# panuelosj/polystokes

Measured on AMD Instinct MI355X. Metric: Stokes-solve wall ms/step (assembly+PCG) on 256^3 grid; CG iters/sec, lower is better.
Workload: dtype f64; 1 GPU; synthetic lid-driven cavity 256x256x256, reduced tiles (tile=16, pad=2), jacobi-PCG, tol 1e-3; parallelism=1 GPU

## Files before the change

### polystokes_amd/__init__.py

```python
import ctypes as C
import os
import subprocess

import numpy as np

from . import _abi
from ._abi import (FieldsIn, FieldsOut, Params, Scene, Stats, default_params)

_HERE = os.path.dirname(os.path.abspath(__file__))
LIB_PATH = os.environ.get("PS_LIB") or os.path.join(_HERE, "libpolystokes_hip.so")
_lib = None

EXPORTED_SYMBOLS = [
    "ps_abi_version", "ps_reduced_dof", "ps_context_create", "ps_context_destroy", "ps_last_error", "ps_params_default",
    "ps_upload_fields", "ps_step_device", "ps_setup_device", "ps_solve_device", "ps_download_fields",
    "polystokes_step", "ps_apply_operator", "ps_apply_preconditioner", "ps_query_array", "ps_read_array",
    "ps_export_component_matrices", "ps_export_matrices", "ps_export_stats", "ps_bench_kernel", "ps_memory_stats", "ps_set_interrupt", "ps_solve_exported_system",
    "ps_set_slab", "ps_set_brick", "ps_comm_unique_id", "ps_comm_init_rccl", "ps_comm_selftest", "ps_comm_init_tcp", "ps_dist_stats",
    "ps_group_create", "ps_group_destroy", "ps_group_rank", "ps_group_step",
    "ps_set_warm_start", "ps_download_solution_fields", "ps_upload_density_field", "ps_set_surface_tension",
    "ps_set_solid_boundary", "ps_set_rheology", "ps_set_solve_precision",
    "ps_upload_fields_device", "ps_upload_density_field_device", "ps_download_fields_device", "ps_download_solution_fields_device",
    "ps_step_device_fields",
]
# ... 144 lines not shown
        put = lambda a: _hip.DeviceBuffer.from_numpy(to_layout(a, layout), pad)
        self.layout, self.host = layout, scene
        for k in ("nx", "ny", "nz", "dx", "dt", "density", "name", "surface_tension"):
            setattr(self, k, getattr(scene, k))
        self.vel = [put(a) for a in scene.vel]
        self.collisionvel = [put(a) for a in scene.collisionvel]
        self.surface, self.collision, self.viscosity = put(scene.surface), put(scene.collision), put(scene.viscosity)
        self.weights = None if scene.weights is None else [put(a) for a in scene.weights]
        self.density_field = None if scene.density_field is None else put(scene.density_field)


def device_scene(scene, layout=_abi.LAYOUT_X_FASTEST, pad=0):
    return DeviceScene(scene, layout, pad)


def fields_in_device(fields):
    fi = FieldsIn()
    fi.nx, fi.ny, fi.nz = fields.nx, fields.ny, fields.nz
    fi.dx, fi.dt = fields.dx, fields.dt
    fi.orig[0] = fi.orig[1] = fi.orig[2] = 0.0
    fi.density = fields.density
    cv = getattr(fields, "collisionvel", None)
    for a in range(3):
        fi.vel[a] = device_address(fields.vel[a])
        fi.collisionvel[a] = device_address(cv[a]) if cv is not None else None
    fi.surface, fi.collision, fi.viscosity = (device_address(fields.surface), device_address(fields.collision),
                                              device_address(fields.viscosity))
    w = getattr(fields, "weights", None)
    for i in range(14):
        fi.weights[i] = device_address(w[i]) if w is not None else None
    return fi


_DT = {(1, "i"): np.int8, (4, "i"): np.int32, (4, "f"): np.float32, (8, "f"): np.float64, (4, "u"): np.uint32}


def _kind(name):
    if name.endswith(("Labels", "Indices", ".col", ".ptr", "Region", "Perm", ".chunkInfo", ".chunkRep", ".code")) or name.startswith("faceRow"):
        return "i"
    if name in ("valuesCoded", "columns16", "diagonalsCoded", "fusedStep", "streamRuns", "rowPerLane", "chebInner32", "warmStartUsed", "densityField", "launchWalk",
                "surfaceTensionReducedFaces", "solidBoundary", "solidSlipEdges", "rheologyModel", "rheologyIterations",
                "solvePrecisionUsed", "solvePassIterations"):
        return "i"
    if name in ("ownedX", "ownedY", "ownedZ"):
        return "f"
    if False:
        return "i"
    if name == "reducedRowFace":
        return "u"
    return "f"


def process_memory_stats():
    v = (C.c_int64 * 4)()
    lib().ps_memory_stats(None, v)
    return {"live_bytes": int(v[0]), "peak_bytes": int(v[1]), "contexts": int(v[3])}


class PolyStokesError(RuntimeError):
    pass


class Solver:

    def __init__(self, device=0, _handle=None):
        self.L = lib()
        self._owned = _handle is None
        h = self.L.ps_context_create(device) if _handle is None else _handle
        if not h:
            raise PolyStokesError(self.L.ps_last_error(None).decode())
        self.h = C.c_void_p(h)
        self.stats = Stats()
        self.scene = None

    def close(self):
        if getattr(self, "h", None):
            if self._owned:
                self.L.ps_context_destroy(self.h)
            self.h = None

    def set_interrupt(self, fn):
# ... 366 lines not shown
```

### polystokes_amd/csrc/ps_blocks.hip

```cpp
#include "ps_context.hpp"
#include "ps_setup_util.hpp"

using namespace ps;

namespace {

constexpr int BS = SETUP_BS;

struct BlockArgs {
    Grid g;
    double invDx;
    const float* lw[7];
    const float* fw[7];
    const int32_t* lab[7];
    const int32_t* act[7];
    const int32_t* reg[7];
    const int32_t* sys[7];
    const int32_t* sysT[3];
    const int32_t* faceRow[3];
    const float* vel[3];
    const float* cvel[3];
    CellField visc;
    FaceDensity dens;
    int64_t nP, nA, faceOff[3];
// ... 72 lines not shown

__device__ inline int skinFaceLen(const BlockArgs& A, int axis, int r, int i, int j, int k) {
    const int3 fd = A.g.dims(1 + axis);
    if (oob3(fd, i, j, k)) return 0;
    const int64_t c = lin3(fd, i, j, k);
    if (A.reg[1 + axis][c] != r || A.lab[1 + axis][c] != PS_REDUCED) return 0;
    int32_t cols[8];
    double vals[8];
    return faceEntries(A, axis, make_int3(i, j, k), cols, vals);
}
__device__ inline unsigned long long blockScanExclPacked(unsigned long long v, unsigned long long* total) {
    __shared__ unsigned long long waveSums64[BS / 64];
    const int lane = threadIdx.x & 63, w = threadIdx.x >> 6;
    unsigned long long incl = v;
#pragma unroll
    for (int o = 1; o < 64; o <<= 1) {
        const unsigned lo = __shfl_up((unsigned)(incl & 0xffffffffull), o, 64), hi = __shfl_up((unsigned)(incl >> 32), o, 64);
        if (lane >= o) incl += ((unsigned long long)hi << 32) | lo;
    }
    if (lane == 63) waveSums64[w] = incl;
    __syncthreads();
    unsigned long long base = 0, tot = 0;
#pragma unroll
    for (int i = 0; i < BS / 64; ++i) { if (i < w) base += waveSums64[i]; tot += waveSums64[i]; }
    __syncthreads();
    *total = tot;
    return base + incl - v;
}
constexpr int SKIN_LONG_MIN = 3;
template <bool ASSIGN>
__global__ void __launch_bounds__(BS) k_skin(BlockArgs A, const int32_t* __restrict__ bbox, const int32_t* __restrict__ itemRegion,
                                             const int32_t* __restrict__ itemStart, int32_t* __restrict__ itemCount, int32_t* __restrict__ faceRow0,
                                             int32_t* __restrict__ faceRow1, int32_t* __restrict__ faceRow2, uint32_t* __restrict__ rrowFace,
                                             int32_t* __restrict__ rrowRegion, int32_t* __restrict__ itemLong) {
    __shared__ unsigned char codes[ASSIGN ? FB_CHUNK : 1];
    const int item = blockIdx.x;
    const int r = itemRegion[item], start = itemStart[item];
    if (A.regionOwned && !A.regionOwned[r]) {
        if (!ASSIGN && threadIdx.x == 0) itemCount[item] = 0;
        if (ASSIGN && threadIdx.x == 0) itemLong[item] = 0;
        return;
    }
    const int bx0 = bbox[r * 6 + 0], by0 = bbox[r * 6 + 1], bz0 = bbox[r * 6 + 2];
    const int ex = bbox[r * 6 + 3] - bx0 + 2, ey = bbox[r * 6 + 4] - by0 + 2, ez = bbox[r * 6 + 5] - bz0 + 2;
    const int total = ex * ey * ez;
    const int end = min(start + FB_CHUNK, total);
    unsigned long long mine = 0;
    for (int base = start; base < end; base += BS) {
        const int pos = base + threadIdx.x;
        if (pos < end) {
            const int i = bx0 + pos % ex, j = by0 + (pos / ex) % ey, k = bz0 + pos / (ex * ey);
            int code = 0;
#pragma unroll
            for (int a = 0; a < 3; ++a) {
                const int n = skinFaceLen(A, a, r, i, j, k);
                if (n > 0) { const bool lg = n >= SKIN_LONG_MIN; code |= (lg ? 2 : 1) << (2 * a); mine += 1ull << (10 * ((lg ? 0 : 3) + a)); }
            }
            if (ASSIGN) codes[pos - start] = (unsigned char)code;
        }
    }
    int catBase[6] = {0, 0, 0, 0, 0, 0};
    if (ASSIGN) {
        int itemTot[6] = {0, 0, 0, 0, 0, 0};
        for (int base = start; base < end; base += BS) {
            const int pos = base + threadIdx.x;
            unsigned long long v = 0;
            if (pos < end) {
                const int code = codes[pos - start];
#pragma unroll
                for (int a = 0; a < 3; ++a) { const int q = (code >> (2 * a)) & 3; if (q) v += 1ull << (10 * ((q == 2 ? 0 : 3) + a)); }
            }
            unsigned long long bt;
            blockScanExclPacked(v, &bt);
#pragma unroll
            for (int c = 0; c < 6; ++c) itemTot[c] += (int)((bt >> (10 * c)) & 1023ull);
        }
        int run = itemCount[item];
#pragma unroll
        for (int c = 0; c < 6; ++c) { catBase[c] = run; run += itemTot[c]; }
        if (threadIdx.x == 0) itemLong[item] = itemTot[0] + itemTot[1] + itemTot[2];
        for (int base = start; base < end; base += BS) {
            const int pos = base + threadIdx.x;
            unsigned long long v = 0;
            int code = 0;
            if (pos < end) {
                code = codes[pos - start];
#pragma unroll
                for (int a = 0; a < 3; ++a) { const int q = (code >> (2 * a)) & 3; if (q) v += 1ull << (10 * ((q == 2 ? 0 : 3) + a)); }
            }
            unsigned long long bt;
            const unsigned long long off = blockScanExclPacked(v, &bt);
// ... 227 lines not shown
    const double visc = (double)A.visc.sample(A.g, (float)q.x + ox, (float)q.y + oy, (float)q.z + oz);
    const double invVisc = clampd(1. / visc, 0., 1e10);
    uInv[t] = A.own.sample(4 + ea, q.x, q.y, q.z) ? 2. * invVisc * vw : 0.;
    if (uDiag) uDiag[t] = 0.5 * visc * clampd(1. / vw, 0., 1.e2);
}

BlockArgs makeArgs(ps_context* c) {
    BlockArgs A;
    A.g = c->g; A.invDx = c->invDx;
    for (int s = 0; s < 7; ++s) {
        A.lw[s] = c->liquidW[s].p; A.fw[s] = c->fluidW[s].p;
        A.lab[s] = c->labels[s].p; A.act[s] = c->activeIdx[s].p; A.reg[s] = c->reducedIdx[s].p; A.sys[s] = c->sysIdx[s].p;
    }
    for (int a = 0; a < 3; ++a) { A.faceRow[a] = c->faceRow[a].p; A.vel[a] = c->vel[a].p; A.cvel[a] = c->cvel[a].p; A.sysT[a] = c->sysIdxT[a].p; }
    A.visc = c->viscSource(); A.dens = c->densSource();
    A.nP = c->nPressures; A.nA = c->nActiveVs;
    A.faceOff[0] = 0; A.faceOff[1] = c->nFace[0]; A.faceOff[2] = c->nFace[0] + c->nFace[1];
    A.own = c->own();
    A.valScale = c->valScale;
    A.codeFail = c->counters.p + CTR_CODE_FAIL;
    A.regionOwned = (c->slabEnabled && c->regionCount > 0) ? c->regionOwned.p : nullptr;
    A.freeSlip = c->solidBoundaryUsed == PS_SOLID_FREE_SLIP ? 1 : 0;
    A.slipEdges = A.freeSlip ? c->slipEdges.p : nullptr;
    return A;
}

__global__ void k_chunk_len4(const int32_t* __restrict__ ptr, const int2* __restrict__ chunkRows, int nChunks, int32_t* __restrict__ len4, int32_t* __restrict__ maxLen) {
    const int ch = blockIdx.x * blockDim.x + threadIdx.x;
    if (ch > nChunks) return;
    int n = 0;
    if (ch < nChunks) { const int2 cr = chunkRows[ch]; n = ptr[cr.x + cr.y] - ptr[cr.x]; atomicMax(maxLen, n); }
    len4[ch] = (n + 3) & ~3;
}
__global__ void __launch_bounds__(BS) k_col16_build(const int32_t* __restrict__ ptr, const int32_t* __restrict__ col, const int8_t* __restrict__ code,
                                                    const int2* __restrict__ chunkRows, const int32_t* __restrict__ start4, uint16_t* __restrict__ col16,
                                                    int8_t* __restrict__ code4, int32_t* __restrict__ winBase, int4* __restrict__ chunkInfo,
                                                    uint8_t* __restrict__ len8, int32_t* __restrict__ fail, int32_t* __restrict__ chunkRep, int nChunks) {
    const int lane = threadIdx.x & 63;
    const int chunk = blockIdx.x * (BS / 64) + (int)(threadIdx.x >> 6);
    if (chunk >= nChunks) return;
    if (lane == 0) chunkRep[chunk] = chunk;
    const int2 cr = chunkRows[chunk];
    const int r0 = cr.x;
    const int p0 = ptr[r0], p1 = ptr[r0 + cr.y];
    const int q0 = start4[chunk], q1 = start4[chunk + 1];
    if (lane == 0) chunkInfo[chunk] = make_int4(q0, (p1 - p0) | (cr.y << 16), cr.x, cr.x);
    for (int i = lane; i < cr.y; i += 64) len8[r0 + i] = (uint8_t)(ptr[r0 + i + 1] - ptr[r0 + i]);
    constexpr int SL = 32;
    if (p1 - p0 > SL * 64) { if (lane == 0) *fail = 1; return; }
    int c[SL];
    unsigned open = 0u;
#pragma unroll
    for (int u = 0; u < SL; ++u) {
        const int i = lane + u * 64;
        const bool o = p0 + i < p1;
        c[u] = o ? col[p0 + i] : 0x7fffffff;
        if (o) open |= 1u << u;
        if (q0 + i < q1) { code4[q0 + i] = o ? code[p0 + i] : (int8_t)0; if (!o) col16[q0 + i] = 0; }
    }
    int used = 16;
    for (int w = 0; w < 16; ++w) {
        int m = 0x7fffffff;
#pragma unroll
        for (int u = 0; u < SL; ++u) if ((open >> u) & 1u) m = min(m, c[u]);
        for (int o = 32; o > 0; o >>= 1) m = min(m, __shfl_xor(m, o));
        const int base = m;
        if (base == 0x7fffffff) { used = w; break; }
        if (lane == 0) winBase[(int64_t)chunk * 16 + w] = base;
#pragma unroll
        for (int u = 0; u < SL; ++u)
            if (((open >> u) & 1u) && c[u] - base < 4096) {
                col16[q0 + lane + u * 64] = (uint16_t)((w << 12) | (c[u] - base));
                open &= ~(1u << u);
            }
    }
    if (lane == 0) for (int w = used; w < 16; ++w) winBase[(int64_t)chunk * 16 + w] = 0;
    if (open) *fail = 1;
}
__global__ void __launch_bounds__(64) k_chunk_hash(const int4* __restrict__ chunkInfo, const uint16_t* __restrict__ col16, const int8_t* __restrict__ code4,
                                                   const uint8_t* __restrict__ len8, unsigned long long* __restrict__ hash, int weak) {
    const int chunk = blockIdx.x;
    const int4 ci = chunkInfo[chunk];
    const int n4 = ((ci.y & 0xffff) + 3) & ~3, rows = (int)((unsigned)ci.y >> 16);
    unsigned long long h = 0;
    if (!weak)
    for (int i = threadIdx.x; i < n4; i += 64)
        h += mix64(((unsigned long long)i << 32) | ((unsigned long long)col16[ci.x + i] << 8) | (uint8_t)code4[ci.x + i]);
    if (!weak)
    for (int i = threadIdx.x; i < rows; i += 64) h += mix64(0x4000000000000000ull | ((unsigned long long)i << 32) | len8[ci.z + i]);
    for (int o = 32; o > 0; o >>= 1) h += __shfl_down(h, o, 64);
    if (threadIdx.x == 0) {
        h = mix64(h ^ (((unsigned long long)(unsigned)n4 << 32) | (unsigned)rows));
        hash[chunk] = h == HASH_EMPTY ? 0ull : h;
    }
}
__global__ void k_chunk_rep_insert(const unsigned long long* __restrict__ hash, int nChunks, unsigned long long* __restrict__ keys, int32_t* __restrict__ vals, unsigned mask) {
    const int chunk = blockIdx.x * blockDim.x + threadIdx.x;
    if (chunk >= nChunks) return;
    const unsigned long long h = hash[chunk];
    hashInsertMin(keys, vals, mask, (unsigned)(h >> 17) & mask, h, chunk);
}
__global__ void __launch_bounds__(64) k_chunk_share(const unsigned long long* __restrict__ hash, const unsigned long long* __restrict__ keys, const int32_t* __restrict__ vals,
                                                    unsigned mask, int4* __restrict__ chunkInfo, const uint16_t* __restrict__ col16, const int8_t* __restrict__ code4,
                                                    const uint8_t* __restrict__ len8, const uint8_t* __restrict__ rowCode, int codeRows,
                                                    unsigned long long* __restrict__ uniqueLen, int32_t* __restrict__ chunkRep) {
    const int chunk = blockIdx.x;
    const unsigned long long h = hash[chunk];
    unsigned slot = (unsigned)(h >> 17) & mask;
    while (keys[slot] != h) slot = (slot + 1) & mask;
    const int rep = vals[slot];
    const int4 ci = chunkInfo[chunk];
    const int n = ci.y & 0xffff, n4 = (n + 3) & ~3, rows = (int)((unsigned)ci.y >> 16);
    bool same = rep != chunk;
    if (same) {
        const int4 cr = chunkInfo[rep];
        same = cr.y == ci.y;
        if (same) {
            for (int i = threadIdx.x; i < n4; i += 64) same = same && col16[ci.x + i] == col16[cr.x + i] && code4[ci.x + i] == code4[cr.x + i];
            for (int i = threadIdx.x; i < rows; i += 64) {
                same = same && len8[ci.z + i] == len8[cr.z + i];
                if (rowCode) {
                    const bool a = ci.z + i < codeRows, b = cr.z + i < codeRows;
                    same = same && a == b && (!a || rowCode[ci.z + i] == rowCode[cr.z + i]);
                }
            }
        }
        same = __all(same) != 0;
        if (same && threadIdx.x == 0) { chunkInfo[chunk].x = cr.x; chunkInfo[chunk].w = cr.z; chunkRep[chunk] = rep; }
    }
    if (!same && threadIdx.x == 0) atomicAdd(uniqueLen, (unsigned long long)n4);
}
__global__ void __launch_bounds__(BS) k_val4_build(const int32_t* __restrict__ ptr, const double* __restrict__ val,
                                                   const int4* __restrict__ chunkInfo, double* __restrict__ val4) {
    const int chunk = blockIdx.x;
    const int4 ci = chunkInfo[chunk];
    const int p0 = ptr[ci.z], n = ci.y & 0xffff, q0 = ci.x;
    const int n4 = (n + 3) & ~3;
    for (int i = threadIdx.x; i < n4; i += BS) val4[q0 + i] = i < n ? val[p0 + i] : 0.;
}
__device__ inline int ellCodeWidth(int W) { return W > 4 ? 8 : (W > 0 ? 4 : 0); }
constexpr int32_t ELL_NULL_BASE = 0x1ffff000;
__global__ void __launch_bounds__(BS) k_ell_plan(const int4* __restrict__ chunkInfo, const uint8_t* __restrict__ len8, const int32_t* __restrict__ chunkRep,
                                                 int32_t* __restrict__ colLen, int32_t* __restrict__ codeLen, int32_t* __restrict__ wpack, int32_t* __restrict__ fail) {
    __shared__ int wmax[BS / 64];
    const int chunk = blockIdx.x;
    const int4 ci = chunkInfo[chunk];
    const int rows = (int)((unsigned)ci.y >> 16);
    int len = (int)threadIdx.x < rows ? (int)len8[ci.z + threadIdx.x] : 0;
    for (int o = 32; o > 0; o >>= 1) len = max(len, __shfl_down(len, o, 64));
    if ((threadIdx.x & 63) == 0) wmax[threadIdx.x >> 6] = len;
    __syncthreads();
    if (threadIdx.x == 0) {
        int cl = 0, vl = 0, wp = 0;
        for (int u = 0; u < BS / 64; ++u) {
            const int W = (wmax[u] + 1) & ~1;
            if (W > 8) *fail = 1;
            cl += 64 * W; vl += 64 * ellCodeWidth(W); wp |= (W & 15) << (4 * u);
        }
// ... 99 lines not shown
        bool ok = !plain && cuts.size() >= 2 && cuts.front() == 0 && (int64_t)cuts.back() == M.rows;
        for (size_t i = 1; ok && i < cuts.size(); ++i) ok = cuts[i] >= cuts[i - 1];
        auto emit = [&](int64_t lo, int64_t hi) { for (int64_t r = lo; r < hi; r += BS) rowsOf.push_back(make_int2((int)r, (int)std::min<int64_t>(BS, hi - r))); };
        if (!ok) emit(0, M.rows);
        else {
            int64_t runLo = 0;
            for (size_t i = 0; i + 1 < cuts.size(); ++i) {
                const int64_t lo = cuts[i], hi = cuts[i + 1];
                if (hi - lo >= CHUNK_ALIGN_MIN) { emit(runLo, lo); emit(lo, hi); runLo = hi; }
            }
            emit(runLo, M.rows);
        }
    }
    const int nChunks = (int)rowsOf.size();
    DevBuf<int2>& chunkRows = scrChunkRows;
    chunkRows.alloc((size_t)nChunks);
    HIP_CHECK(hipMemcpyAsync(chunkRows.p, rowsOf.data(), (size_t)nChunks * sizeof(int2), hipMemcpyHostToDevice, stream));
    DevBuf<int32_t>& start4 = scrStart4;
    start4.alloc((size_t)nChunks + 1);
    HIP_CHECK(hipMemsetAsync(counters.p + CTR_CHUNK_MAX, 0, sizeof(int32_t), stream));
    hipLaunchKernelGGL(k_chunk_len4, dim3(gridFor(nChunks + 1, BS)), dim3(BS), 0, stream, M.ptr.p, (const int2*)chunkRows.p, nChunks, start4.p, counters.p + CTR_CHUNK_MAX);
    const int64_t total4 = exclusiveScanI32(start4.p, nChunks + 1);
    if (total4 < 0) return;
    const int maxLen = readCounter(CTR_CHUNK_MAX);
    M.nv = std::max(1, (maxLen + 4 * BS - 1) / (4 * BS));
    if (M.nv > 2) return;
    if ((uint64_t)std::max(M.rows, M.cols) * 8 >= 0xffffffffull || (uint64_t)total4 * 2 >= 0xffffffffull) return;
    M.streamLen = total4;
    M.uniqueLen = total4;
    M.nChunks = nChunks;
    M.col16.alloc((size_t)total4 + 8); M.code4.alloc((size_t)total4 + 8);
    M.winBase.alloc((size_t)nChunks * 16); M.chunkInfo.alloc((size_t)nChunks); M.len8.alloc((size_t)M.rows); M.chunkRep.alloc((size_t)nChunks);
    HIP_CHECK(hipMemsetAsync(counters.p + slot, 0, sizeof(int32_t), stream));
    hipLaunchKernelGGL(k_col16_build, dim3((unsigned)((nChunks + BS / 64 - 1) / (BS / 64))), dim3(BS), 0, stream, M.ptr.p, M.col.p, M.code.p, (const int2*)chunkRows.p, start4.p, M.col16.p,
                       M.code4.p, M.winBase.p, M.chunkInfo.p, M.len8.p, counters.p + slot, M.chunkRep.p, nChunks);
    M.col16ok = readCounter(slot) == 0;
    if (M.col16ok && !M.packed) buildVal4(M);
    static const bool noShare = envInt(PS_ENV("PS_NO_SHARED_RUNS"), 0) != 0;
    static const bool weakHash = envInt(PS_ENV("PS_WEAK_CHUNK_HASH"), 0) != 0;
    if (M.col16ok && M.packed && shareRuns && !noShare && nChunks > 1) {
        unsigned cap = 1024;
        while (cap < 4u * (unsigned)nChunks) cap <<= 1;
        DevBuf<unsigned long long>& hash = scrHash; DevBuf<unsigned long long>& keys = scrKeys; DevBuf<unsigned long long>& uniq = scrUniq;
        DevBuf<int32_t>& vals = scrVals;
        hash.alloc((size_t)nChunks); keys.alloc(cap); vals.alloc(cap); uniq.alloc(1);
        HIP_CHECK(hipMemsetAsync(keys.p, 0xff, (size_t)cap * 8, stream));
        HIP_CHECK(hipMemsetAsync(vals.p, 0x7f, (size_t)cap * 4, stream));
        HIP_CHECK(hipMemsetAsync(uniq.p, 0, 8, stream));
        hipLaunchKernelGGL(k_chunk_hash, dim3((unsigned)nChunks), dim3(64), 0, stream, (const int4*)M.chunkInfo.p, (const uint16_t*)M.col16.p, (const int8_t*)M.code4.p,
                           (const uint8_t*)M.len8.p, hash.p, weakHash ? 1 : 0);
        hipLaunchKernelGGL(k_chunk_rep_insert, dim3(gridFor(nChunks, BS)), dim3(BS), 0, stream, (const unsigned long long*)hash.p, nChunks, keys.p, vals.p, cap - 1);
        hipLaunchKernelGGL(k_chunk_share, dim3((unsigned)nChunks), dim3(64), 0, stream, (const unsigned long long*)hash.p, (const unsigned long long*)keys.p,
                           (const int32_t*)vals.p, cap - 1, M.chunkInfo.p, (const uint16_t*)M.col16.p, (const int8_t*)M.code4.p, (const uint8_t*)M.len8.p, rowCode, codeRows, uniq.p, M.chunkRep.p);
        unsigned long long u = 0;
        HIP_CHECK(hipMemcpyAsync(&u, uniq.p, 8, hipMemcpyDeviceToHost, stream));
        HIP_CHECK(hipStreamSynchronize(stream));
        M.uniqueLen = (int64_t)u;
    }
    if (PS_ENV_VERBOSE()) std::fprintf(stderr, "[polystokes] compressed stream: rows %lld nnz %lld, %d chunks, fullest %d (nv %d), ok %d, distinct runs hold %lld of %lld entries\n",
                                           (long long)M.rows, (long long)M.nnz, nChunks, maxLen, M.nv, (int)M.col16ok, (long long)M.uniqueLen, (long long)M.streamLen);
}

namespace {
constexpr unsigned long long DICT_EMPTY = 0xfff8dead0000beefull;
__device__ inline int dictHash(unsigned long long k) { k ^= k >> 33; k *= 0xff51afd7ed558ccdull; k ^= k >> 29; return (int)(k & 255ull); }
__global__ void __launch_bounds__(BS) k_dict_build(const double* __restrict__ v, int64_t n, unsigned long long* __restrict__ table, int32_t* __restrict__ overflow) {
    __shared__ unsigned long long snap[256];
    snap[threadIdx.x] = __hip_atomic_load(&table[threadIdx.x], __ATOMIC_RELAXED, __HIP_MEMORY_SCOPE_AGENT);
    __syncthreads();
    const int64_t stride = (int64_t)gridDim.x * blockDim.x;
    const int64_t rounds = (n + stride - 1) / stride;
    for (int64_t k = 0; k < rounds; ++k) {
        const int64_t i = k * stride + (int64_t)blockIdx.x * blockDim.x + threadIdx.x;
        const bool have = i < n;
        const unsigned long long key = have ? (unsigned long long)__double_as_longlong(v[i]) : 0ull;
        bool miss = have;
        if (have && key == DICT_EMPTY) { *overflow = 1; miss = false; }
        if (miss) {
            const int h0 = dictHash(key);
            for (int probe = 0; probe < 256; ++probe) {
                const unsigned long long cur = snap[(h0 + probe) & 255];
                if (cur == key) { miss = false; break; }
                if (cur == DICT_EMPTY) break;
// ... 58 lines not shown
        cutsS = blockStartRow;
        for (size_t r = 1; r < skinCutsHost.size(); ++r) cutsS.push_back((int32_t)(nActiveVs + skinCutsHost[r]));
    }
    if (!blockStartSys.empty() && (int64_t)blockStartSys.back() == nSystem) cutsT = blockStartSys;
    shareRuns = share;
    buildCol16(S, CTR_COL16_FAIL_S, cutsS, mcCoded ? mcCode.p : nullptr, (int)nActiveVs);
    buildCol16(St, CTR_COL16_FAIL_ST, cutsT, uCoded ? uCode.p : nullptr, (int)nSystem);
    if (share) { buildEll(S); buildEll(St); } else S.ellok = St.ellok = false;
}

void ps_context::constructMatrixBlocks() {
    nActiveVs = nFace[0] + nFace[1] + nFace[2];
    nReducedVs = regionCount * PS_RD;
    nPressures = nCenter;
    nStresses = 3 * nCenter + nEdge[0] + nEdge[1] + nEdge[2];
    nSystem = nPressures + nStresses;
    nTotalDOFs = nActiveVs + nReducedVs + nPressures + nStresses;
    if (nSystem >= 0x7fffffff || nActiveVs >= 0x7fffffff) throw Error("system too large for 32-bit DOF indices");

    valScale = invDx / 64.;
    HIP_CHECK(hipMemsetAsync(counters.p + CTR_CODE_FAIL, 0, sizeof(int32_t), stream));
    solidBoundaryUsed = solidBoundarySet;
    if (solidBoundaryUsed == PS_SOLID_FREE_SLIP) {
        slipEdges.alloc(1);
        HIP_CHECK(hipMemsetAsync(slipEdges.p, 0, sizeof(int32_t), stream));
    }
    buildInternalNumbering();
    haloForward = false;
    buildHaloLists();
    BlockArgs A = makeArgs(this);
    nReducedRows = 0;
    maxRegionRows = 0;
    if (regionCount > 0 && sbItems > 0) {
        hipLaunchKernelGGL(k_skin<false>, dim3((unsigned)sbItems), dim3(BS), 0, stream, A, bbox.p, sbItemRegion.p, sbItemStart.p, sbItemCount.p,
                           faceRow[0].p, faceRow[1].p, faceRow[2].p, (uint32_t*)nullptr, (int32_t*)nullptr, (int32_t*)nullptr);
        HIP_CHECK(hipMemsetAsync(sbItemCount.p + sbItems, 0, sizeof(int32_t), stream));
        nReducedRows = exclusiveScanI32(sbItemCount.p, sbItems + 1);
        rrowFace.alloc((size_t)nReducedRows);
        rrowRegion.alloc((size_t)nReducedRows);
        sbItemLong.alloc((size_t)sbItems);
        hipLaunchKernelGGL(k_skin<true>, dim3((unsigned)sbItems), dim3(BS), 0, stream, A, bbox.p, sbItemRegion.p, sbItemStart.p, sbItemCount.p,
                           faceRow[0].p, faceRow[1].p, faceRow[2].p, rrowFace.p, rrowRegion.p, sbItemLong.p);
        std::vector<int32_t> itemOff((size_t)sbItems + 1), itemLong((size_t)sbItems);
        HIP_CHECK(hipMemcpyAsync(itemOff.data(), sbItemCount.p, itemOff.size() * 4, hipMemcpyDeviceToHost, stream));
        HIP_CHECK(hipMemcpyAsync(itemLong.data(), sbItemLong.p, itemLong.size() * 4, hipMemcpyDeviceToHost, stream));
        HIP_CHECK(hipStreamSynchronize(stream));
        skinCutsHost.clear();
        for (int64_t q = 0; q < sbItems; ++q) {
            skinCutsHost.push_back(itemOff[(size_t)q]);
            if (itemLong[(size_t)q] > 0 && itemOff[(size_t)q] + itemLong[(size_t)q] < itemOff[(size_t)q + 1]) skinCutsHost.push_back(itemOff[(size_t)q] + itemLong[(size_t)q]);
        }
        skinCutsHost.push_back(itemOff[(size_t)sbItems]);
        std::vector<int32_t>& rptr = hostTab[6]; std::vector<int32_t>& cR = hostTab[7]; std::vector<int32_t>& cS = hostTab[8]; std::vector<int32_t>& cE = hostTab[9];
        std::vector<int32_t>& cptr = hostTab[10];
        rptr.assign((size_t)regionCount + 1, 0); cR.clear(); cS.clear(); cE.clear(); cptr.assign((size_t)regionCount + 1, 0);
        for (int64_t r = 0; r <= regionCount; ++r) rptr[(size_t)r] = itemOff[(size_t)sbRegionItemPtrHost[(size_t)r]];
        regionRowPtrHost = rptr;
        for (int64_t r = 0; r < regionCount; ++r) {
            cptr[(size_t)r] = (int32_t)cR.size();
            const int32_t lo = rptr[(size_t)r], hi = rptr[(size_t)r + 1], len = hi - lo;
            maxRegionRows = std::max<int64_t>(maxRegionRows, len);
            if (len > 0) {
                const int32_t pieces = (len + RC_ROWS - 1) / RC_ROWS;
                for (int32_t q = 0; q < pieces; ++q) {
                    cR.push_back((int32_t)r);
                    cS.push_back(lo + (int32_t)((int64_t)len * q / pieces));
                    cE.push_back(lo + (int32_t)((int64_t)len * (q + 1) / pieces));
                }
            }
        }
        cptr[(size_t)regionCount] = (int32_t)cR.size();
        nRChunks = (int64_t)cR.size();
        regionRowPtr.alloc(rptr.size()); rchunkRegion.alloc(cR.size()); rchunkStart.alloc(cS.size()); rchunkEnd.alloc(cE.size());
        regionChunkPtr.alloc(cptr.size());
        HIP_CHECK(hipMemcpyAsync(regionRowPtr.p, rptr.data(), rptr.size() * 4, hipMemcpyHostToDevice, stream));
// ... 88 lines not shown
```

### polystokes_amd/csrc/ps_context.hip

```cpp
#include <algorithm>
#include <chrono>
#include <cstdio>
#include <cstring>
#include <ctime>
#include <fstream>

#include "ps_context.hpp"
#include "ps_setup_util.hpp"

using namespace ps;

namespace {

struct StageTimer {
    hipEvent_t ev[PS_STAGE_COUNT + 1];
    hipStream_t s;
    int n = 0;
    explicit StageTimer(hipStream_t st) : s(st) {
        for (auto& e : ev) HIP_CHECK(hipEventCreate(&e));
    }
    ~StageTimer() { for (auto& e : ev) (void)hipEventDestroy(e); }
    void mark(int i) { HIP_CHECK(hipEventRecord(ev[i], s)); }
    double ms(int a, int b) { float f = 0; HIP_CHECK(hipEventElapsedTime(&f, ev[a], ev[b])); return f; }
};
// ... 350 lines not shown
    }
    regHost("solidBoundary", &solidBoundaryUsed, 1, 4);
    if (solidBoundaryUsed == PS_SOLID_FREE_SLIP) reg("solidSlipEdges", slipEdges.p, 1, 4);
    regHost("rheologyModel", &rheoModelUsed, 1, 4);
    if (rheoModelUsed != PS_RHEOLOGY_NEWTONIAN) {
        reg("rheologyStrainRate", rheoRate.p, g.count(0), 4);
        reg("rheologyViscosity", rheoMu.p, g.count(0), 4);
        regHost("rheologyIterations", rheoIters.data(), (int64_t)rheoIters.size(), 4);
    }
    if (P.preconditioner == PS_PRE_DIAGONAL) regp("dinv", dinv.p, nSystem, permSys.p, 0);
    if (isSolved) {
        regp("recoveredActiveVelocity", recovered.p, nActiveVs, permRow.p, 0);
        reg("recoveredReducedVelocity", recovered.p ? recovered.p + nActiveVs : nullptr, nReducedVs, 8);
    }
    regHost("valuesCoded", &valuesCodedHost, 1, 4);
    diagFlagsHost = (uCoded ? 1 : 0) | (mcCoded ? 2 : 0);
    regHost("diagonalsCoded", &diagFlagsHost, 1, 4);
    regHost("columns16", &columns16Host, 1, 4);
    regHost("fusedStep", &fusedStepHost, 1, 4);
    regHost("launchWalk", launchWalkHost, 5 * LAUNCH_WALK_FIELDS, 4);
    chebInner32Host = chebInner32 ? 1 : 0;
    regHost("chebInner32", &chebInner32Host, 1, 4);
    streamRunsHost[0] = S.col16ok ? (int32_t)S.uniqueLen : 0; streamRunsHost[1] = S.col16ok ? (int32_t)S.streamLen : 0;
    streamRunsHost[2] = St.col16ok ? (int32_t)St.uniqueLen : 0; streamRunsHost[3] = St.col16ok ? (int32_t)St.streamLen : 0;
    regHost("streamRuns", streamRunsHost, 4, 4);
    rowPerLaneHost[0] = ((S.ellok && S.packed) ? 1 : 0) | ((St.ellok && St.packed) ? 2 : 0); rowPerLaneHost[1] = ilPlaneMajor;
    regHost("rowPerLane", rowPerLaneHost, 2, 4);
    reg("sysPerm", permSys.p, nSystem, 4);
    reg("rowPerm", permRow.p, nActiveVs, 4);
    reg("S.ptr", S.ptr.p, S.rows + 1, 4); reg("S.col", S.col.p, S.nnz, 4); reg("S.val", S.val.p, S.nnz, 8);
    reg("St.ptr", St.ptr.p, St.rows + 1, 4); reg("St.col", St.col.p, St.nnz, 4); reg("St.val", St.val.p, St.nnz, 8);
    if (S.col16ok) { reg("S.chunkInfo", S.chunkInfo.p, (int64_t)S.nChunks * 4, 4); reg("S.chunkRep", S.chunkRep.p, S.nChunks, 4); }
    if (St.col16ok) { reg("St.chunkInfo", St.chunkInfo.p, (int64_t)St.nChunks * 4, 4); reg("St.chunkRep", St.chunkRep.p, St.nChunks, 4); }
    if (S.packed) reg("S.code", S.code.p, S.nnz, 1);
    if (St.packed) reg("St.code", St.code.p, St.nnz, 1);
    reg("reducedRowFace", rrowFace.p, nReducedRows, 4);
    reg("reducedRowRegion", rrowRegion.p, nReducedRows, 4);
    static const char* ax[3] = {"X", "Y", "Z"};
    for (int a = 0; a < 3; ++a) {
        reg(std::string("vel") + ax[a], velOut[a].p, g.count(1 + a), 4);
        reg(std::string("valid") + ax[a], valid[a].p, g.count(1 + a), 4);
        reg(std::string("faceRow") + ax[a], faceRow[a].p, g.count(1 + a), 4);
        if (slabEnabled && isSolved) reg(std::string("owned") + ax[a], ownedFace[a].p, g.count(1 + a), 4);
    }
}

#define PS_TRY(ctx, ...)                                                     \
    ps::SinkScope sinkScope_((ctx) ? &(ctx)->deferred : nullptr);            \
    try { __VA_ARGS__ } catch (const ps::Error& e) {                         \
        if (ctx) { (ctx)->err = e.msg; (ctx)->drainDeferred(false); }        \
        return PS_FAILED;                                                    \
    } catch (const std::exception& e) {                                      \
        if (ctx) { (ctx)->err = e.what(); (ctx)->drainDeferred(false); }     \
        return PS_FAILED;                                                    \
    }

static std::string g_createError;

static bool writeMarketVector(const std::string& fn, const std::vector<double>& v) {
    std::ofstream out(fn.c_str(), std::ios::out);
    if (!out) return false;
    out.flags(std::ios_base::scientific);
    out.precision(17);
    out << "%%MatrixMarket matrix array real general\n";
    out << v.size() << " " << 1 << "\n";
    for (double d : v) out << d << "\n";
// ... 753 lines not shown
```

### polystokes_amd/csrc/ps_context.hpp

```cpp
#pragma once
#include <map>
#include <memory>

#include "ps_common.hpp"

namespace ps {

struct DevCSR {
    int64_t rows = 0, cols = 0, nnz = 0;
    DevBuf<int32_t> ptr;
    DevBuf<int32_t> col;
    DevBuf<double> val;
    DevBuf<int8_t> code;
    bool packed = false;
    DevBuf<uint16_t> col16;
    DevBuf<int8_t> code4;
    DevBuf<double> val4;
    DevBuf<int32_t> winBase;
    DevBuf<int4> chunkInfo;
    DevBuf<uint8_t> len8;
    DevBuf<int32_t> chunkRep;
    int nChunks = 0;
    int64_t uniqueLen = 0;
    bool col16ok = false;
// ... 297 lines not shown

    int solveIterations = -1;
    double solveError = -1;
    int usedBiCGStab = 0;
    ps_stats lastStats{};

    std::map<std::string, ps::ArrayInfo> arrays;
    std::map<std::string, std::vector<char>> hostArrays;

    void upload(const ps_params* p, const ps_fields_in* in);
    void buildIntegrationWeightsAlt();
    void classifyCells();
    void constructReducedRegions();
    void constructOnlyActiveRegions();
    void classifyFaces();
    void classifyEdges();
    void constructCenterReducedIndices(int part);
    void constructFacesReducedIndices();
    void constructEdgesReducedIndices();
    void constructActiveIndices();
    void buildValidFaces();
    void computeRegionBoxes();
    void computeCenterOfMasses();
    void computeLeastSquaresFits();
    void computeReducedMassMatrices();
    void computeReducedViscosityMatricesInteriorOnly();
    void assembleReducedBlocks();
    void constructMatrixBlocks();
    void buildCol16(ps::DevCSR& M, ps::Counter failSlot, const std::vector<int32_t>& cuts, const uint8_t* rowCode, int codeRows);
    void buildEll(ps::DevCSR& M);
    void buildStreams(bool share);
    bool shareRuns = true;
    ps::DevBuf<int2> scrChunkRows; ps::DevBuf<int32_t> scrSlice, scrStart4, scrVals, scrKeep, scrRemap, scrEllCol, scrEllCode, scrEllW; ps::DevBuf<unsigned long long> scrHash, scrKeys, scrUniq;
    void ensureValues(ps::DevCSR& M);
    void buildVal4(ps::DevCSR& M);
    std::vector<int32_t> regionRowPtrHost;
    std::vector<int32_t> hostTab[20];
    void assembleSystemPressureStressFactored();
    void constructPreconditioner();
    int solve();
    void estimateLambdaMax();
    void applyPreconditionerDevice(const double* r, double* z, double* scratch);
    int chebyshevApply(const double* rvec, double* zA, double* zB, double* rzPartial, const ps::CGScalars* sc, bool firstDone = false, double** zOut = nullptr);
    double chebTheta() const;
    int ntLevel() const;
    int solveEigenCG();
    void constructGuessVectors();
    void buildExplicitA(std::vector<int64_t>& ptr, std::vector<int32_t>& col, std::vector<double>& val);
    void recoverVelocityFromPressureStress();
    void applySolutionToVelocity();
    void applyOperator(const double* x, double* y, double* dotPartialsOut);

    int setup(ps_stats* stats);
    void setupPhase(int phase);
    std::shared_ptr<void> setupState;
    int setupPhaseDone = -1;
    int solveStage(ps_stats* stats);
    void fillDimData(ps_stats* st) const;
    void registerArrays();

    int32_t orderedIndexAssign(int s, int mode, ps::DevBuf<int32_t>& out, int counterSlot = -1);
    int64_t interleavedIndexAssign(int ngroups, const int* samples, const int* weights, int32_t* const* outs);
    int64_t interleavedIndexAssignEx(int ngroups, const int* samples, const int* weights, int32_t* const* outs, bool ownFilter,
                                     int64_t* ownedRange);
    void buildInternalNumbering();
    int64_t exclusiveScanI32(int32_t* data, int64_t n, int counterSlot = -1);
// ... 18 lines not shown
```

Baseline: 1006 ms/step.

## Cache skin codes across passes and fuse chunk hashing into col16 build

The skin classification pass now writes per-cell face codes to a global scratch buffer, and the assign pass reads them back instead of recomputing skinFaceLen for every cell. The col16 build kernel now loads columns and codes four at a time, writes col16 and code4 with packed vector stores, and computes the chunk hash inline, which removes the separate k_chunk_hash launch. The chunk-share comparison now checks packed 32-bit words. In exchange it adds a scratch allocation of sbItems*FB_CHUNK bytes, uses unaligned vector loads, and sets a waves-per-EU occupancy hint. It also registers the stream arrays for export.

```diff
diff --git a/polystokes_amd/__init__.py b/polystokes_amd/__init__.py
--- a/polystokes_amd/__init__.py
+++ b/polystokes_amd/__init__.py
@@ -200,11 +200,11 @@
     return fi
 
 
-_DT = {(1, "i"): np.int8, (4, "i"): np.int32, (4, "f"): np.float32, (8, "f"): np.float64, (4, "u"): np.uint32}
+_DT = {(1, "i"): np.int8, (4, "i"): np.int32, (4, "f"): np.float32, (8, "f"): np.float64, (4, "u"): np.uint32, (2, "u"): np.uint16, (1, "u"): np.uint8}
 
 
 def _kind(name):
-    if name.endswith(("Labels", "Indices", ".col", ".ptr", "Region", "Perm", ".chunkInfo", ".chunkRep", ".code")) or name.startswith("faceRow"):
+    if name.endswith(("Labels", "Indices", ".col", ".ptr", "Region", "Perm", ".chunkInfo", ".chunkRep", ".code", ".code4", ".winBase")) or name.startswith("faceRow"):
         return "i"
     if name in ("valuesCoded", "columns16", "diagonalsCoded", "fusedStep", "streamRuns", "rowPerLane", "chebInner32", "warmStartUsed", "densityField", "launchWalk",
                 "surfaceTensionReducedFaces", "solidBoundary", "solidSlipEdges", "rheologyModel", "rheologyIterations",
@@ -214,7 +214,7 @@
         return "f"
     if False:
         return "i"
-    if name == "reducedRowFace":
+    if name == "reducedRowFace" or name.endswith((".col16", ".len8")):
         return "u"
     return "f"
 
diff --git a/polystokes_amd/csrc/ps_blocks.hip b/polystokes_amd/csrc/ps_blocks.hip
--- a/polystokes_amd/csrc/ps_blocks.hip
+++ b/polystokes_amd/csrc/ps_blocks.hip
@@ -128,8 +128,9 @@
 __global__ void __launch_bounds__(BS) k_skin(BlockArgs A, const int32_t* __restrict__ bbox, const int32_t* __restrict__ itemRegion,
                                              const int32_t* __restrict__ itemStart, int32_t* __restrict__ itemCount, int32_t* __restrict__ faceRow0,
                                              int32_t* __restrict__ faceRow1, int32_t* __restrict__ faceRow2, uint32_t* __restrict__ rrowFace,
-                                             int32_t* __restrict__ rrowRegion, int32_t* __restrict__ itemLong) {
+                                             int32_t* __restrict__ rrowRegion, int32_t* __restrict__ itemLong, unsigned char* __restrict__ skinCodes) {
     __shared__ unsigned char codes[ASSIGN ? FB_CHUNK : 1];
+    unsigned char* __restrict__ itemCodes = skinCodes + (size_t)blockIdx.x * FB_CHUNK;
     const int item = blockIdx.x;
     const int r = itemRegion[item], start = itemStart[item];
     if (A.regionOwned && !A.regionOwned[r]) {
@@ -145,6 +146,7 @@
     for (int base = start; base < end; base += BS) {
         const int pos = base + threadIdx.x;
         if (pos < end) {
+            if (ASSIGN) { codes[pos - start] = itemCodes[pos - start]; continue; }
             const int i = bx0 + pos % ex, j = by0 + (pos / ex) % ey, k = bz0 + pos / (ex * ey);
             int code = 0;
 #pragma unroll
@@ -152,7 +154,7 @@
                 const int n = skinFaceLen(A, a, r, i, j, k);
                 if (n > 0) { const bool lg = n >= SKIN_LONG_MIN; code |= (lg ? 2 : 1) << (2 * a); mine += 1ull << (10 * ((lg ? 0 : 3) + a)); }
             }
-            if (ASSIGN) codes[pos - start] = (unsigned char)code;
+            itemCodes[pos - start] = (unsigned char)code;
         }
     }
     int catBase[6] = {0, 0, 0, 0, 0, 0};
@@ -446,10 +448,17 @@
     if (ch < nChunks) { const int2 cr = chunkRows[ch]; n = ptr[cr.x + cr.y] - ptr[cr.x]; atomicMax(maxLen, n); }
     len4[ch] = (n + 3) & ~3;
 }
-__global__ void __launch_bounds__(BS) k_col16_build(const int32_t* __restrict__ ptr, const int32_t* __restrict__ col, const int8_t* __restrict__ code,
+struct __attribute__((packed, aligned(4))) Col4 { int32_t v[4]; };
+__device__ inline unsigned long long chunkHashFinish(unsigned long long h, int n4, int rows) {
+    h = mix64(h ^ (((unsigned long long)(unsigned)n4 << 32) | (unsigned)rows));
+    return h == HASH_EMPTY ? 0ull : h;
+}
+__global__ void __launch_bounds__(BS) __attribute__((amdgpu_waves_per_eu(5)))
+k_col16_build(const int32_t* __restrict__ ptr, const int32_t* __restrict__ col, const int8_t* __restrict__ code,
                                                     const int2* __restrict__ chunkRows, const int32_t* __restrict__ start4, uint16_t* __restrict__ col16,
                                                     int8_t* __restrict__ code4, int32_t* __restrict__ winBase, int4* __restrict__ chunkInfo,
-                                                    uint8_t* __restrict__ len8, int32_t* __restrict__ fail, int32_t* __restrict__ chunkRep, int nChunks) {
+                                                    uint8_t* __restrict__ len8, int32_t* __restrict__ fail, int32_t* __restrict__ chunkRep, int nChunks,
+                                                    unsigned long long* __restrict__ hash, int weak) {
     const int lane = threadIdx.x & 63;
     const int chunk = blockIdx.x * (BS / 64) + (int)(threadIdx.x >> 6);
     if (chunk >= nChunks) return;
@@ -459,19 +468,47 @@
     const int p0 = ptr[r0], p1 = ptr[r0 + cr.y];
     const int q0 = start4[chunk], q1 = start4[chunk + 1];
     if (lane == 0) chunkInfo[chunk] = make_int4(q0, (p1 - p0) | (cr.y << 16), cr.x, cr.x);
-    for (int i = lane; i < cr.y; i += 64) len8[r0 + i] = (uint8_t)(ptr[r0 + i + 1] - ptr[r0 + i]);
-    constexpr int SL = 32;
-    if (p1 - p0 > SL * 64) { if (lane == 0) *fail = 1; return; }
+    const bool hashed = hash != nullptr && !weak;
+    unsigned long long h = 0;
+#pragma unroll
+    for (int k = 0; k < BS / 64; ++k) {
+        const int i = lane + k * 64;
+        if (i < cr.y) {
+            const int len = ptr[r0 + i + 1] - ptr[r0 + i];
+            len8[r0 + i] = (uint8_t)len;
+            if (hashed) h += mix64(0x4000000000000000ull | ((unsigned long long)i << 32) | (uint8_t)len);
+        }
+    }
+    constexpr int SL = 32, SG = SL / 4;
+    const int n = p1 - p0;
+    if (n > SL * 64) { if (lane == 0) *fail = 1; return; }
     int c[SL];
+    unsigned cpk[SG];
     unsigned open = 0u;
 #pragma unroll
-    for (int u = 0; u < SL; ++u) {
-        const int i = lane + u * 64;
-        const bool o = p0 + i < p1;
-        c[u] = o ? col[p0 + i] : 0x7fffffff;
-        if (o) open |= 1u << u;
-        if (q0 + i < q1) { code4[q0 + i] = o ? code[p0 + i] : (int8_t)0; if (!o) col16[q0 + i] = 0; }
-    }
+    for (int g = 0; g < SG; ++g) {
+        const int i0 = 4 * lane + 256 * g;
+        cpk[g] = 0u;
+#pragma unroll
+        for (int k = 0; k < 4; ++k) c[4 * g + k] = 0x7fffffff;
+        if (i0 + 3 < n) {
+            const Col4 t = *reinterpret_cast<const Col4*>(col + p0 + i0);
+#pragma unroll
+            for (int k = 0; k < 4; ++k) c[4 * g + k] = t.v[k];
+            __builtin_memcpy(&cpk[g], code + p0 + i0, 4);
+            open |= 0xfu << (4 * g);
+        } else {
+#pragma unroll
+            for (int k = 0; k < 4; ++k)
+                if (i0 + k < n) {
+                    c[4 * g + k] = col[p0 + i0 + k];
+                    cpk[g] |= (unsigned)(uint8_t)code[p0 + i0 + k] << (8 * k);
+                    open |= 1u << (4 * g + k);
+                }
+        }
+        if (q0 + i0 < q1) *reinterpret_cast<unsigned*>(code4 + q0 + i0) = cpk[g];
+    }
+    const unsigned had = open;
     int used = 16;
     for (int w = 0; w < 16; ++w) {
         int m = 0x7fffffff;
@@ -484,28 +521,28 @@
 #pragma unroll
         for (int u = 0; u < SL; ++u)
             if (((open >> u) & 1u) && c[u] - base < 4096) {
-                col16[q0 + lane + u * 64] = (uint16_t)((w << 12) | (c[u] - base));
+                c[u] = (w << 12) | (c[u] - base);
                 open &= ~(1u << u);
             }
     }
     if (lane == 0) for (int w = used; w < 16; ++w) winBase[(int64_t)chunk * 16 + w] = 0;
     if (open) *fail = 1;
-}
-__global__ void __launch_bounds__(64) k_chunk_hash(const int4* __restrict__ chunkInfo, const uint16_t* __restrict__ col16, const int8_t* __restrict__ code4,
-                                                   const uint8_t* __restrict__ len8, unsigned long long* __restrict__ hash, int weak) {
-    const int chunk = blockIdx.x;
-    const int4 ci = chunkInfo[chunk];
-    const int n4 = ((ci.y & 0xffff) + 3) & ~3, rows = (int)((unsigned)ci.y >> 16);
-    unsigned long long h = 0;
-    if (!weak)
-    for (int i = threadIdx.x; i < n4; i += 64)
-        h += mix64(((unsigned long long)i << 32) | ((unsigned long long)col16[ci.x + i] << 8) | (uint8_t)code4[ci.x + i]);
-    if (!weak)
-    for (int i = threadIdx.x; i < rows; i += 64) h += mix64(0x4000000000000000ull | ((unsigned long long)i << 32) | len8[ci.z + i]);
-    for (int o = 32; o > 0; o >>= 1) h += __shfl_down(h, o, 64);
-    if (threadIdx.x == 0) {
-        h = mix64(h ^ (((unsigned long long)(unsigned)n4 << 32) | (unsigned)rows));
-        hash[chunk] = h == HASH_EMPTY ? 0ull : h;
+#pragma unroll
+    for (int g = 0; g < SG; ++g) {
+        const int i0 = 4 * lane + 256 * g;
+        if (q0 + i0 < q1) {
+            unsigned v[4];
+#pragma unroll
+            for (int k = 0; k < 4; ++k) {
+                v[k] = ((had >> (4 * g + k)) & 1u) ? ((unsigned)c[4 * g + k] & 0xffffu) : 0u;
+                if (hashed) h += mix64(((unsigned long long)(i0 + k) << 32) | ((unsigned long long)v[k] << 8) | ((cpk[g] >> (8 * k)) & 0xffu));
+            }
+            *reinterpret_cast<uint2*>(col16 + q0 + i0) = make_uint2(v[0] | (v[1] << 16), v[2] | (v[3] << 16));
+        }
+    }
+    if (hash) {
+        for (int o = 32; o > 0; o >>= 1) h += __shfl_down(h, o, 64);
+        if (lane == 0) hash[chunk] = chunkHashFinish(h, q1 - q0, cr.y);
     }
 }
 __global__ void k_chunk_rep_insert(const unsigned long long* __restrict__ hash, int nChunks, unsigned long long* __restrict__ keys, int32_t* __restrict__ vals, unsigned mask) {
@@ -530,14 +567,24 @@
         const int4 cr = chunkInfo[rep];
         same = cr.y == ci.y;
         if (same) {
-            for (int i = threadIdx.x; i < n4; i += 64) same = same && col16[ci.x + i] == col16[cr.x + i] && code4[ci.x + i] == code4[cr.x + i];
+            unsigned diff = 0u;
+            const uint2* __restrict__ a2 = reinterpret_cast<const uint2*>(col16 + ci.x);
+            const uint2* __restrict__ b2 = reinterpret_cast<const uint2*>(col16 + cr.x);
+            const unsigned* __restrict__ a1 = reinterpret_cast<const unsigned*>(code4 + ci.x);
+            const unsigned* __restrict__ b1 = reinterpret_cast<const unsigned*>(code4 + cr.x);
+            for (int i = threadIdx.x; i < n4 / 4; i += 64) {
+                const uint2 a = a2[i], b = b2[i];
+                diff |= (a.x ^ b.x) | (a.y ^ b.y) | (a1[i] ^ b1[i]);
+            }
             for (int i = threadIdx.x; i < rows; i += 64) {
-                same = same && len8[ci.z + i] == len8[cr.z + i];
+                diff |= (unsigned)(len8[ci.z + i] ^ len8[cr.z + i]);
                 if (rowCode) {
                     const bool a = ci.z + i < codeRows, b = cr.z + i < codeRows;
-                    same = same && a == b && (!a || rowCode[ci.z + i] == rowCode[cr.z + i]);
+                    if (a != b) diff |= 1u;
+                    else if (a) diff |= (unsigned)(rowCode[ci.z + i] ^ rowCode[cr.z + i]);
                 }
             }
+            same = diff == 0u;
         }
         same = __all(same) != 0;
         if (same && threadIdx.x == 0) { chunkInfo[chunk].x = cr.x; chunkInfo[chunk].w = cr.z; chunkRep[chunk] = rep; }
@@ -703,23 +750,23 @@
     M.col16.alloc((size_t)total4 + 8); M.code4.alloc((size_t)total4 + 8);
     M.winBase.alloc((size_t)nChunks * 16); M.chunkInfo.alloc((size_t)nChunks); M.len8.alloc((size_t)M.rows); M.chunkRep.alloc((size_t)nChunks);
     HIP_CHECK(hipMemsetAsync(counters.p + slot, 0, sizeof(int32_t), stream));
+    static const bool noShare = envInt(PS_ENV("PS_NO_SHARED_RUNS"), 0) != 0;
+    static const bool weakHash = envInt(PS_ENV("PS_WEAK_CHUNK_HASH"), 0) != 0;
+    const bool wantShare = M.packed && shareRuns && !noShare && nChunks > 1;
+    if (wantShare) scrHash.alloc((size_t)nChunks);
     hipLaunchKernelGGL(k_col16_build, dim3((unsigned)((nChunks + BS / 64 - 1) / (BS / 64))), dim3(BS), 0, stream, M.ptr.p, M.col.p, M.code.p, (const int2*)chunkRows.p, start4.p, M.col16.p,
-                       M.code4.p, M.winBase.p, M.chunkInfo.p, M.len8.p, counters.p + slot, M.chunkRep.p, nChunks);
+                       M.code4.p, M.winBase.p, M.chunkInfo.p, M.len8.p, counters.p + slot, M.chunkRep.p, nChunks, wantShare ? scrHash.p : (unsigned long long*)nullptr, weakHash ? 1 : 0);
     M.col16ok = readCounter(slot) == 0;
     if (M.col16ok && !M.packed) buildVal4(M);
-    static const bool noShare = envInt(PS_ENV("PS_NO_SHARED_RUNS"), 0) != 0;
-    static const bool weakHash = envInt(PS_ENV("PS_WEAK_CHUNK_HASH"), 0) != 0;
-    if (M.col16ok && M.packed && shareRuns && !noShare && nChunks > 1) {
+    if (M.col16ok && wantShare) {
         unsigned cap = 1024;
         while (cap < 4u * (unsigned)nChunks) cap <<= 1;
         DevBuf<unsigned long long>& hash = scrHash; DevBuf<unsigned long long>& keys = scrKeys; DevBuf<unsigned long long>& uniq = scrUniq;
         DevBuf<int32_t>& vals = scrVals;
-        hash.alloc((size_t)nChunks); keys.alloc(cap); vals.alloc(cap); uniq.alloc(1);
+        keys.alloc(cap); vals.alloc(cap); uniq.alloc(1);
         HIP_CHECK(hipMemsetAsync(keys.p, 0xff, (size_t)cap * 8, stream));
         HIP_CHECK(hipMemsetAsync(vals.p, 0x7f, (size_t)cap * 4, stream));
         HIP_CHECK(hipMemsetAsync(uniq.p, 0, 8, stream));
-        hipLaunchKernelGGL(k_chunk_hash, dim3((unsigned)nChunks), dim3(64), 0, stream, (const int4*)M.chunkInfo.p, (const uint16_t*)M.col16.p, (const int8_t*)M.code4.p,
-                           (const uint8_t*)M.len8.p, hash.p, weakHash ? 1 : 0);
         hipLaunchKernelGGL(k_chunk_rep_insert, dim3(gridFor(nChunks, BS)), dim3(BS), 0, stream, (const unsigned long long*)hash.p, nChunks, keys.p, vals.p, cap - 1);
         hipLaunchKernelGGL(k_chunk_share, dim3((unsigned)nChunks), dim3(64), 0, stream, (const unsigned long long*)hash.p, (const unsigned long long*)keys.p,
                            (const int32_t*)vals.p, cap - 1, M.chunkInfo.p, (const uint16_t*)M.col16.p, (const int8_t*)M.code4.p, (const uint8_t*)M.len8.p, rowCode, codeRows, uniq.p, M.chunkRep.p);
@@ -844,15 +891,16 @@
     nReducedRows = 0;
     maxRegionRows = 0;
     if (regionCount > 0 && sbItems > 0) {
+        scrSkinCodes.alloc((size_t)sbItems * FB_CHUNK);
         hipLaunchKernelGGL(k_skin<false>, dim3((unsigned)sbItems), dim3(BS), 0, stream, A, bbox.p, sbItemRegion.p, sbItemStart.p, sbItemCount.p,
-                           faceRow[0].p, faceRow[1].p, faceRow[2].p, (uint32_t*)nullptr, (int32_t*)nullptr, (int32_t*)nullptr);
+                           faceRow[0].p, faceRow[1].p, faceRow[2].p, (uint32_t*)nullptr, (int32_t*)nullptr, (int32_t*)nullptr, scrSkinCodes.p);
         HIP_CHECK(hipMemsetAsync(sbItemCount.p + sbItems, 0, sizeof(int32_t), stream));
         nReducedRows = exclusiveScanI32(sbItemCount.p, sbItems + 1);
         rrowFace.alloc((size_t)nReducedRows);
         rrowRegion.alloc((size_t)nReducedRows);
         sbItemLong.alloc((size_t)sbItems);
         hipLaunchKernelGGL(k_skin<true>, dim3((unsigned)sbItems), dim3(BS), 0, stream, A, bbox.p, sbItemRegion.p, sbItemStart.p, sbItemCount.p,
-                           faceRow[0].p, faceRow[1].p, faceRow[2].p, rrowFace.p, rrowRegion.p, sbItemLong.p);
+                           faceRow[0].p, faceRow[1].p, faceRow[2].p, rrowFace.p, rrowRegion.p, sbItemLong.p, scrSkinCodes.p);
         std::vector<int32_t> itemOff((size_t)sbItems + 1), itemLong((size_t)sbItems);
         HIP_CHECK(hipMemcpyAsync(itemOff.data(), sbItemCount.p, itemOff.size() * 4, hipMemcpyDeviceToHost, stream));
         HIP_CHECK(hipMemcpyAsync(itemLong.data(), sbItemLong.p, itemLong.size() * 4, hipMemcpyDeviceToHost, stream));
diff --git a/polystokes_amd/csrc/ps_context.hip b/polystokes_amd/csrc/ps_context.hip
--- a/polystokes_amd/csrc/ps_context.hip
+++ b/polystokes_amd/csrc/ps_context.hip
@@ -406,6 +406,12 @@
     reg("St.ptr", St.ptr.p, St.rows + 1, 4); reg("St.col", St.col.p, St.nnz, 4); reg("St.val", St.val.p, St.nnz, 8);
     if (S.col16ok) { reg("S.chunkInfo", S.chunkInfo.p, (int64_t)S.nChunks * 4, 4); reg("S.chunkRep", S.chunkRep.p, S.nChunks, 4); }
     if (St.col16ok) { reg("St.chunkInfo", St.chunkInfo.p, (int64_t)St.nChunks * 4, 4); reg("St.chunkRep", St.chunkRep.p, St.nChunks, 4); }
+    auto regStream = [&](const std::string& n, const ps::DevCSR& M) {
+        reg(n + ".col16", M.col16.p, M.streamLen, 2); reg(n + ".code4", M.code4.p, M.streamLen, 1);
+        reg(n + ".winBase", M.winBase.p, (int64_t)M.nChunks * 16, 4); reg(n + ".len8", M.len8.p, M.rows, 1);
+    };
+    if (S.col16ok) regStream("S", S);
+    if (St.col16ok) regStream("St", St);
     if (S.packed) reg("S.code", S.code.p, S.nnz, 1);
     if (St.packed) reg("St.code", St.code.p, St.nnz, 1);
     reg("reducedRowFace", rrowFace.p, nReducedRows, 4);
diff --git a/polystokes_amd/csrc/ps_context.hpp b/polystokes_amd/csrc/ps_context.hpp
--- a/polystokes_amd/csrc/ps_context.hpp
+++ b/polystokes_amd/csrc/ps_context.hpp
@@ -353,6 +353,7 @@
     void buildStreams(bool share);
     bool shareRuns = true;
     ps::DevBuf<int2> scrChunkRows; ps::DevBuf<int32_t> scrSlice, scrStart4, scrVals, scrKeep, scrRemap, scrEllCol, scrEllCode, scrEllW; ps::DevBuf<unsigned long long> scrHash, scrKeys, scrUniq;
+    ps::DevBuf<unsigned char> scrSkinCodes;
     void ensureValues(ps::DevCSR& M);
     void buildVal4(ps::DevCSR& M);
     std::vector<int32_t> regionRowPtrHost;
```

Result: no change. 1003 ms/step (median of 6 runs) (-0.3%).
